# bababyVN/medical-image-segmentation-and-classification

Measured on AMD Instinct MI355X. Metric: images/sec (train step) Attention U-Net 256x256 bs=32/GPU, higher is better.
Workload: dtype bf16; 1 GPU; AttentionUNet 256x256 train step (fwd+BCE+bwd+clip+AdamW), bs=32/GPU, NHWC bf16 activations, fp32 master weights; global_batch=32, parallelism=dp1, hip_graph=False, wgrad_side_stream=True, plan_replay=C (mi355_plan_run)

## Files before the change

### include/mi355conv.h

```cpp
#ifndef MI355CONV_H_
#define MI355CONV_H_

#include <stdint.h>

#ifdef __cplusplus
extern "C" {
#endif

typedef struct ihipStream_t* mi355_stream_t;

enum { MI355_F32 = 0, MI355_BF16 = 1, MI355_F16 = 2 };
enum { MI355_OK = 0, MI355_ERR_ARG = -1, MI355_ERR_UNSUPPORTED = -2, MI355_ERR_RUNTIME = -3 };

int mi355_version(void);
const char* mi355_last_error(void);


int mi355_pack_input_nchw(const float* x, void* y, int N, int C, int H, int W, int Cpad, int dtype,
                          mi355_stream_t s);
int mi355_pack_input_im2col3(const float* x, void* y, int N, int C, int H, int W, int dtype, mi355_stream_t s);
int mi355_unpack_output_nchw(const void* x, float* y, int N, int C, int H, int W, int ld, int dtype,
                             mi355_stream_t s);
int mi355_pack_nchw(const float* x, void* y, int N, int C, int H, int W, int ld, int dtype, mi355_stream_t s);

// ... 6 lines not shown
int mi355_conv2d_igemm(const void* in, const void* wk, const float* bias, void* out,
                       int N, int Hi, int Wi, int Ci, int ldi,
                       int Ho, int Wo, int Co, int ldo,
                       int KH, int KW, int mul, int kmul, int off, int div, int up,
                       int accumulate, float* stats, int dtype, mi355_stream_t s);
int mi355_conv2d_igemm_variant(int Hi, int Wi, int Ci, int Ho, int Wo, int Co, int KH, int KW, int mul, int kmul, int off,
                               int div, int up, int dtype);
int mi355_conv2d_igemm_variant_n(int N, int Hi, int Wi, int Ci, int Ho, int Wo, int Co, int KH, int KW, int mul, int kmul,
                                 int off, int div, int up, int dtype);
int mi355_conv2d_igemm_dma_tile(int N, int Ho, int Wo, int Ci, int Co);
int mi355_conv2d_igemm_generic_tile(int N, int Ho, int Wo, int Co);
int mi355_conv2d_igemm_stat_rows(int N, int Hi, int Wi, int Ci, int Ho, int Wo, int Co, int KH, int KW,
                                 int mul, int kmul, int off, int div, int up, int dtype);
int mi355_conv2d_igemm_pool2_ok(int N, int Hi, int Wi, int Ci, int Ho, int Wo, int Co, int KH, int KW,
                                int mul, int kmul, int off, int div, int up, int dtype);
const char* mi355_conv2d_igemm_kernel_name(int N, int Hi, int Wi, int Ci, int Ho, int Wo, int Co, int KH, int KW,
                                           int mul, int kmul, int off, int div, int up, int dtype);

int mi355_conv2d_wgrad_splits(int N, int Ho, int Wo, int Ci, int Co, int KH, int KW);
int mi355_conv2d_wgrad_variant(int N, int Ho, int Wo, int KH, int KW, int stride, int pad, int dtype);
const char* mi355_conv2d_wgrad_kernel_name(int N, int Ho, int Wo, int Ci, int Co, int KH, int KW, int stride, int pad, int dtype);
int mi355_conv2d_wgrad(const void* x, const void* dy, float* ws, int splits,
                       int N, int Hi, int Wi, int Ci, int ldx,
                       int Ho, int Wo, int Co, int ldy,
                       int KH, int KW, int stride, int pad, int up, int dtype, mi355_stream_t s);
int mi355_conv2d_wgrad_multi_ok(int N, int Ho, int Wo, int dtype);
int mi355_conv2d_wgrad_multi(const void* x0, const void* dy0, const void* x1, const void* dy1, const void* x2, const void* dy2,
                             const void* x3, const void* dy3, const void* x4, const void* dy4, const void* x5, const void* dy5,
                             int napp, float* ws, int splits, int N, int Hi, int Wi, int Ci, int ldx, int Ho, int Wo, int Co,
                             int ldy, int up, int dtype, mi355_stream_t s);
// ... 256 lines not shown
```

### medical-image-segmentation-and-classification_amd/csrc/conv3x3_halo.hpp

```cpp
#pragma once
#include <type_traits>

#include "common.hpp"
#include "conv3x3_tile.hpp"

template <int TH, int TW> struct HaloRwCfg {
  static constexpr int BN = 64;
  static constexpr int NPIX = (TH + 2) * (TW + 2);
  static constexpr int P_INSTR = (NPIX + 15) / 16;
  static constexpr int PATCH_BYTES = P_INSTR * 1024;
  static constexpr int STAGE_BYTES = 3 * BN * 64;
  static constexpr int NS = 3;
  static constexpr int RING = 2 * PATCH_BYTES + NS * STAGE_BYTES;
  static constexpr int C_BYTES = TH * TW * (BN * 2 + 16);
  static constexpr int EPI_BYTES = C_BYTES + 2 * 2 * BN * 4;
  static constexpr int LDS_BYTES = RING > EPI_BYTES ? RING : EPI_BYTES;
};

template <typename T, int TH, int TW>
__global__ __launch_bounds__(256, 2) void conv3x3_halo_rw_kernel(const ConvArgs a) {
  static_assert(sizeof(T) == 2, "bf16 / fp16 only");
  typedef HaloRwCfg<TH, TW> Cfg;
  constexpr int BN = 64, BK = 32, EPC = 8, BM = TH * TW;
  static_assert(BM == 256 && TW % 16 == 0, "tile must hold 256 pixels in rows of 16-pixel blocks");
  constexpr int PH = TH + 2, PW = TW + 2, NPIX = PH * PW;
  constexpr int PIXB = BK * 2;
  constexpr int P_INSTR = Cfg::P_INSTR;
  constexpr int P_IT = (P_INSTR + 3) / 4;
  constexpr int PATCH_BYTES = Cfg::PATCH_BYTES;
  constexpr int SLAB = BN * PIXB, STAGE = Cfg::STAGE_BYTES, NS = Cfg::NS;
  constexpr int B_IT = 3;
  constexpr int WM = 2, WN = 2, WTM = BM / WM, WTN = BN / WN;
  constexpr int RW = WTM / TW, XB = TW / 16;
  constexpr int MB = RW * XB, NB = WTN / 16;
  constexpr int C_PITCH = BN * 2 + 16;
  extern __shared__ __attribute__((aligned(16))) unsigned char lds[];
// ... 159 lines not shown
    }
    if constexpr (STATS) {
#pragma unroll
      for (int nb = 0; nb < NB; ++nb)
#pragma unroll
        for (int r = 0; r < 4; ++r) {
          const float s1 = row16_sum(sm[nb][r >> 1][r & 1]), s2 = row16_sum(sq[nb][r >> 1][r & 1]);
          if (l16 == 0) {
            red[(wm * 2 + 0) * BN + wn * WTN + nb * 16 + 4 * c4 + r] = s1;
            red[(wm * 2 + 1) * BN + wn * WTN + nb * 16 + 4 * c4 + r] = s2;
          }
        }
    }
  };
  using Yes = std::true_type;
  if (a.stats) {
    if (a.relu) finish(Yes{}, Yes{}); else finish(No{}, Yes{});
  } else {
    if (a.relu) finish(Yes{}, No{}); else finish(No{}, No{});
  }
  __syncthreads();
  fold_tile_stats<WM, BN>(a, red, tid, tile);
  constexpr int CPRC = BN / EPC;
  if (a.pool2) {
    const int Ho2 = a.Ho >> 1, Wo2 = a.Wo >> 1;
    for (int id = tid; id < (BM / 4) * CPRC; id += 256) {
      const int g = id / CPRC, c = id - g * CPRC;
      const int gy = g / (TW / 2), gx = g - gy * (TW / 2);
      float sum[EPC];
#pragma unroll
      for (int e = 0; e < EPC; ++e) sum[e] = 0.f;
#pragma unroll
      for (int dy = 0; dy < 2; ++dy)
#pragma unroll
        for (int dx = 0; dx < 2; ++dx) {
          const int row = (2 * gy + dy) * TW + 2 * gx + dx;
          const Vec16<T> v = *reinterpret_cast<const Vec16<T>*>(lds + row * C_PITCH + c * 16);
// ... 4 lines not shown
      Vec16<T> v;
      if (a.accumulate) {
        const Vec16<T> o = ld16<T>(p);
#pragma unroll
        for (int e = 0; e < EPC; ++e) v.v[e] = from_f32<T>(sum[e] + to_f32<T>(o.v[e]));
      } else {
#pragma unroll
        for (int e = 0; e < EPC; ++e) v.v[e] = from_f32<T>(sum[e]);
      }
      st16<T>(p, v);
    }
    return;
  }
  constexpr int NST = BM * CPRC / 256;
  static_assert(NST * 256 == BM * CPRC, "whole store rounds");
  auto addr = [&](int it) __attribute__((always_inline)) {
    const int id = tid + it * 256, row = id / CPRC, c = id - row * CPRC;
    const int py = row / TW, px = row - py * TW;
    return out + ((size_t)(n * a.Ho + y0 + py) * a.Wo + x0 + px) * a.ldo + n0 + c * EPC;
  };
  if (a.accumulate) {
    Vec16<T> old[NST];
#pragma unroll
    for (int it = 0; it < NST; ++it) old[it] = ld16<T>(addr(it));
#pragma unroll
    for (int it = 0; it < NST; ++it) {
      const int id = tid + it * 256, row = id / CPRC, c = id - row * CPRC;
      Vec16<T> v = *reinterpret_cast<const Vec16<T>*>(lds + row * C_PITCH + c * 16);
#pragma unroll
      for (int e = 0; e < EPC; ++e) v.v[e] = from_f32<T>(to_f32<T>(v.v[e]) + to_f32<T>(old[it].v[e]));
      st16<T>(addr(it), v);
    }
  } else {
#pragma unroll
    for (int it = 0; it < NST; ++it) {
      const int id = tid + it * 256, row = id / CPRC, c = id - row * CPRC;
      st16<T>(addr(it), *reinterpret_cast<const Vec16<T>*>(lds + row * C_PITCH + c * 16));
    }
  }
}

template <typename T, int TH, int TW>
static int launch_halo_rw(const ConvArgs& a, hipStream_t s) {
  const int grid = a.N * (a.Ho / TH) * (a.Wo / TW) * (a.Co / 64);
  return launch_with_lds<conv3x3_halo_rw_kernel<T, TH, TW>, HaloRwCfg<TH, TW>::LDS_BYTES>("conv3x3_halo_rw", grid, 256, s, a);
}
```

### medical-image-segmentation-and-classification_amd/csrc/conv3x3_halo_pp128.hpp

```cpp
#pragma once
#include <type_traits>

#include "common.hpp"
#include "conv3x3_tile.hpp"

struct HaloPp128Cfg {
  static constexpr int TH = 16, TW = 32, HTH = 8, BN = 128;
  static constexpr int PWL = 36;
  static constexpr int NPIX = (TH + 2) * PWL;
  static constexpr int P_INSTR = (NPIX + 15) / 16;
  static constexpr int PATCH_BYTES = P_INSTR * 1024;
  static constexpr int STAGE_BYTES = 3 * BN * 64;
  static constexpr int NS = 3;
  static constexpr int NPB = 2;
  static constexpr int RING = NPB * PATCH_BYTES + NS * STAGE_BYTES;
  static constexpr int C_BYTES = HTH * TW * (BN * 2 + 16);
  static constexpr int EPI_BYTES = 2 * C_BYTES + 2 * 2 * 2 * BN * 4;
  static constexpr int LDS_BYTES = RING > EPI_BYTES ? RING : EPI_BYTES;
};

template <typename T>
__global__ __launch_bounds__(512) void conv3x3_halo_pp128_kernel(const ConvArgs a) {
  static_assert(sizeof(T) == 2, "bf16 / fp16 only");
  typedef HaloPp128Cfg Cfg;
  constexpr int TH = Cfg::TH, TW = Cfg::TW, HTH = Cfg::HTH;
  constexpr int BN = Cfg::BN, BK = 32, EPC = 8, HBM = HTH * TW;
  constexpr int PW = TW + 2, PWL = Cfg::PWL, NPIX = Cfg::NPIX;
  constexpr int PIXB = BK * 2;
  constexpr int P_INSTR = Cfg::P_INSTR;
  constexpr int P_IT = P_INSTR / 8;
  static_assert(P_INSTR == 8 * P_IT + 1, "one left-over piece");
  constexpr int PATCH_BYTES = Cfg::PATCH_BYTES;
  constexpr int SLAB = BN * PIXB, STAGE = Cfg::STAGE_BYTES;
  constexpr int WN = 2, WTM = HBM / 2, WTN = BN / WN;
  constexpr int RW = HTH, XB = 1;
  constexpr int MB = RW * XB, NB = WTN / 16;
  constexpr int NPR = RW + 2;
  constexpr int C_PITCH = BN * 2 + 16;
// ... 186 lines not shown
      for (int nb = 0; nb < NB; ++nb) t += acc[mb][nb];
    reinterpret_cast<f32x4*>(a.out)[tid + 512 * blockIdx.x] = t;
    return;
  }
#endif
  T* __restrict__ out = reinterpret_cast<T*>(a.out);
  struct alignas(8) Pack4 { T v[4]; };
  unsigned char* const ctile = lds + half * Cfg::C_BYTES;
  float* const red = reinterpret_cast<float*>(lds + 2 * Cfg::C_BYTES);
  auto finish = [&](auto relu_tag, auto stats_tag) __attribute__((always_inline)) {
    constexpr bool RELU = decltype(relu_tag)::value, STATS = decltype(stats_tag)::value;
    f32x2 sm[NB][2], sq[NB][2];
    f32x4 bias4[NB];
#pragma unroll
    for (int nb = 0; nb < NB; ++nb) {
      bias4[nb] = a.bias ? *reinterpret_cast<const f32x4*>(a.bias + n0 + wn * WTN + nb * 16 + 4 * c4) : f32x4{0.f, 0.f, 0.f, 0.f};
#pragma unroll
      for (int j = 0; j < 2; ++j) { sm[nb][j] = f32x2{0.f, 0.f}; sq[nb][j] = f32x2{0.f, 0.f}; }
    }
#pragma unroll
    for (int mb = 0; mb < MB; ++mb) {
      const int row = mb * TW + wm * 16 + l16;
#pragma unroll
      for (int nb = 0; nb < NB; ++nb) {
        Pack4 pk;
#pragma unroll
        for (int r = 0; r < 4; ++r) {
          const float v = acc[mb][nb][r] + bias4[nb][r];
          pk.v[r] = from_f32<T>(RELU ? __builtin_amdgcn_fmed3f(v, 0.f, INFINITY) : v);
        }
        if constexpr (STATS) {
// ... 9 lines not shown
    }
    if constexpr (STATS) {
#pragma unroll
      for (int nb = 0; nb < NB; ++nb)
#pragma unroll
        for (int r = 0; r < 4; ++r) {
          const float s1 = row16_sum(sm[nb][r >> 1][r & 1]), s2 = row16_sum(sq[nb][r >> 1][r & 1]);
          if (l16 == 0) {
            red[((half * 2 + wm) * 2 + 0) * BN + wn * WTN + nb * 16 + 4 * c4 + r] = s1;
            red[((half * 2 + wm) * 2 + 1) * BN + wn * WTN + nb * 16 + 4 * c4 + r] = s2;
          }
        }
    }
  };
  auto finish_any = [&]() __attribute__((always_inline)) {
    if (a.stats) {
      if (a.relu) finish(Yes{}, Yes{}); else finish(No{}, Yes{});
    } else {
      if (a.relu) finish(Yes{}, No{}); else finish(No{}, No{});
    }
  };
  finish_any();
  __syncthreads();
  fold_tile_stats<4, BN>(a, red, tid, tile);
  constexpr int CPRC = BN / EPC;
  constexpr int BM = TH * TW;
  if (a.pool2) {
    const int Ho2 = a.Ho >> 1, Wo2 = a.Wo >> 1;
    for (int id = tid; id < (BM / 4) * CPRC; id += 512) {
      const int g = id / CPRC, c = id - g * CPRC;
      const int gy = g / (TW / 2), gx = g - gy * (TW / 2);
      float sum[EPC];
#pragma unroll
      for (int e = 0; e < EPC; ++e) sum[e] = 0.f;
#pragma unroll
      for (int dy = 0; dy < 2; ++dy)
#pragma unroll
        for (int dx = 0; dx < 2; ++dx) {
          const int row = (2 * gy + dy) * TW + 2 * gx + dx;
          const Vec16<T> v = *reinterpret_cast<const Vec16<T>*>(lds + (row / HBM) * Cfg::C_BYTES + (row % HBM) * C_PITCH + c * 16);
#pragma unroll
// ... 16 lines not shown
  for (int id = tid; id < BM * CPRC; id += 512) {
    const int row = id / CPRC, c = id - row * CPRC;
    const int py = row / TW, px = row - py * TW;
    T* p = out + ((size_t)(n * a.Ho + y0 + py) * a.Wo + x0 + px) * a.ldo + n0 + c * EPC;
    Vec16<T> v = *reinterpret_cast<const Vec16<T>*>(lds + (row / HBM) * Cfg::C_BYTES + (row % HBM) * C_PITCH + c * 16);
    if (a.accumulate) {
      const Vec16<T> o = ld16<T>(p);
#pragma unroll
      for (int e = 0; e < EPC; ++e) v.v[e] = from_f32<T>(to_f32<T>(v.v[e]) + to_f32<T>(o.v[e]));
    }
    st16<T>(p, v);
  }
}

template <typename T>
static int launch_halo_pp128(const ConvArgs& a, hipStream_t s) {
  const int grid = a.N * (a.Ho / HaloPp128Cfg::TH) * (a.Wo / HaloPp128Cfg::TW) * (a.Co / HaloPp128Cfg::BN);
  return launch_with_lds<conv3x3_halo_pp128_kernel<T>, HaloPp128Cfg::LDS_BYTES>("conv3x3_halo_pp128", grid, 512, s, a);
}
```

### medical-image-segmentation-and-classification_amd/csrc/conv3x3_tile.hpp

```cpp
#pragma once
#include "common.hpp"

struct HaloTile { int sp, n, y0, x0, n0; };
template <int TH, int TW, int BN> __device__ __forceinline__ HaloTile halo_tile(const ConvArgs& a) {
  const int NT = a.Co / BN, TXN = a.Wo / TW, TYN = a.Ho / TH;
  int t = xcd_tile(blockIdx.x, gridDim.x);
  const int nt = t % NT; t /= NT;
  const int sp = t;
  const int tx = t % TXN; t /= TXN;
  const int ty = t % TYN;
  return {sp, t / TYN, ty * TH, tx * TW, nt * BN};
}

template <typename T> __device__ __forceinline__ size_t weight_row_offset(int row, size_t wrow, int slot) {
  return (size_t)row * wrow + (slot ^ (((row >> 2) & 1) << 1)) * (16 / sizeof(T));
}
__device__ __forceinline__ int tap_index(bool flip, int ph, int pw) { return flip ? (2 - ph) * 3 + (2 - pw) : ph * 3 + pw; }

template <int ROWS, int BN> __device__ __forceinline__ void fold_tile_stats(const ConvArgs& a, const float* red, int tid, const HaloTile& t) {
  if (a.stats && tid < 2 * BN) {
    const int q = tid / BN, c = tid - q * BN;
    float v = 0.f;
#pragma unroll
    for (int w = 0; w < ROWS; ++w) v += red[(w * 2 + q) * BN + c];
    a.stats[((size_t)t.sp * 2 + q) * a.Co + t.n0 + c] = v;
  }
}

template <auto KERNEL, int LDS_BYTES, typename... Args>
static int launch_with_lds(const char* name, int grid, int block, hipStream_t s, const Args&... args) {
  static const hipError_t configured = hipFuncSetAttribute((const void*)KERNEL, hipFuncAttributeMaxDynamicSharedMemorySize, LDS_BYTES);
  if (configured != hipSuccess) MI355_FAIL((int)configured, "%s: cannot reserve %d B of LDS: %s", name, LDS_BYTES, hipGetErrorString(configured));
  hipLaunchKernelGGL(KERNEL, dim3(grid), dim3(block), LDS_BYTES, s, args...);
  MI355_LAUNCH_CHECK();
  return MI355_OK;
}
```

### medical-image-segmentation-and-classification_amd/csrc/conv_igemm.hip

```cpp
#include "common.hpp"
#include <stdlib.h>

struct ConvArgs {
  const void* in;
  const void* wk;
  const float* bias;
  void* out;
  int N, Hi, Wi, Ci, ldi;
  int Ho, Wo, Co, ldo;
  int KH, KW;
  int mul, kmul, off, dshift, up;
  int accumulate;
  int relu;
  int pool2;
  float* stats;
  int M;
  int HoWo;
  int Hlog, Wlog;
};

template <typename T> struct Frag;
template <> struct Frag<bf16_t> {
  static __device__ __forceinline__ void mma(const uint4& a, const uint4& b, f32x16& c) {
    c = __builtin_amdgcn_mfma_f32_32x32x16_bf16(__builtin_bit_cast(bf16x8, a), __builtin_bit_cast(bf16x8, b), c, 0,
                                                0, 0);
  }
};
template <> struct Frag<f16_t> {
  static __device__ __forceinline__ void mma(const uint4& a, const uint4& b, f32x16& c) {
    c = mfma_32x32x16<f16_t>(__builtin_bit_cast(bf16x8, a), __builtin_bit_cast(bf16x8, b), c);
  }
};
template <> struct Frag<float> {
// ... 476 lines not shown
    return n;
  }();
  return cus;
}
struct Switches {
  int force_generic = getenv("MI355_IGEMM_VARIANT") ? atoi(getenv("MI355_IGEMM_VARIANT")) == 0 : 0;
  int halo_pp = env_int("MI355_HALO_PP", 0);
  int pp128 = env_int("MI355_HALO_PP128", 1), pp128_min_ci = env_int("MI355_HALO_PP128_MINCI", 256);
  int pp128_fill = env_int("MI355_PP128_FILL", 80);
  int ws64 = env_int("MI355_WS64", 1), ws128 = env_int("MI355_WS128", 1);
  long long ws_min_tiles = getenv("MI355_WS64_MIN_TILES") ? atoll(getenv("MI355_WS64_MIN_TILES")) : 4ll * device_cus();
  int ws128_tile_mult = env_int("MI355_WS128_TILE_MULT", 6);
  int gemm256 = env_int("MI355_GEMM256", 1);
  long long gemm256_min_tiles = getenv("MI355_GEMM256_MIN_TILES") ? atoll(getenv("MI355_GEMM256_MIN_TILES")) : 128;
  int dma_smallgrid = env_int("MI355_DMA_SMALLGRID", 1);
};
static const Switches& switches() { static const Switches sw{}; return sw; }

static bool halo_family(IgemmVariant v) {
  return v == IG_HALO_8x32 || v == IG_HALO_16x16 || v == IG_HALO_PP || v == IG_HALO_PP128 || v == IG_WS64 || v == IG_WS128;
}
static bool image_fits_descriptor(int Hi, int Wi, int ldi, int esz) { return (long long)Hi * Wi * ldi * esz < (1ll << 31); }

static int small_grid_tile_n(long long M, int Co, bool to32) {
  const long long rows = (M + 127) / 128;
  int bn = Co % 128 == 0 ? 128 : (Co % 64 == 0 ? 64 : 32);
  if (switches().dma_smallgrid) {
    const int cus = device_cus();
    if (bn == 128 && rows * (Co / 128) * 2 <= cus) bn = 64;
    if (bn == 64 && to32 && rows * (Co / 64) * 2 <= cus) bn = 32;
// ... 113 lines not shown
#undef IG_KERNEL

#define GEOM_PARAMS int Hi, int Wi, int Ci, int Ho, int Wo, int Co, int KH, int KW, int mul, int kmul, int off, int div, int up, int dtype
#define GEOM_SHAPE(N) ConvShape{N, Hi, Wi, Ci, Ho, Wo, Co, KH, KW, mul, kmul, off, div, up, dtype}
extern "C" int mi355_conv2d_igemm_variant(GEOM_PARAMS) { return (int)choose(GEOM_SHAPE(1)).shape_variant; }
extern "C" int mi355_conv2d_igemm_variant_n(int N, GEOM_PARAMS) { return (int)choose(GEOM_SHAPE(N)).variant; }
extern "C" int mi355_conv2d_igemm_stat_rows(int N, GEOM_PARAMS) { return choose(GEOM_SHAPE(N)).stat_rows; }
extern "C" int mi355_conv2d_igemm_pool2_ok(int N, GEOM_PARAMS) { return choose(GEOM_SHAPE(N)).pool2; }
extern "C" int mi355_conv2d_igemm_dma_tile(int N, int Ho, int Wo, int Ci, int Co) { return small_grid_tile_n((long long)N * Ho * Wo, Co, Ci % 64 == 0); }
extern "C" int mi355_conv2d_igemm_generic_tile(int N, int Ho, int Wo, int Co) { return small_grid_tile_n((long long)N * Ho * Wo, Co, true); }
extern "C" const char* mi355_conv2d_igemm_kernel_name(int N, GEOM_PARAMS) {
  static thread_local char name[IG_NAME_LEN];
  const ConvShape s = GEOM_SHAPE(N); const ConvChoice c = choose(s);
  const int rc = dispatch_dtype(dtype, "conv2d_igemm_kernel_name", [&](auto tag) { return launch_or_name<decltype(tag)>(c, conv_args(s), nullptr, name); });
  return rc == MI355_OK ? name : nullptr;
}

extern "C" int mi355_conv2d_igemm(const void* in, const void* wk, const float* bias, void* out, int N, int Hi, int Wi,
                                  int Ci, int ldi, int Ho, int Wo, int Co, int ldo, int KH, int KW, int mul, int kmul,
                                  int off, int div, int up, int accumulate, float* stats, int dtype, mi355_stream_t s) {
  MI355_CHECK_ARG(in && wk && out, "conv2d_igemm: null pointer");
  MI355_CHECK_ARG(N > 0 && Hi > 0 && Wi > 0 && Ho > 0 && Wo > 0 && KH > 0 && KW > 0, "conv2d_igemm: bad extent");
  MI355_CHECK_ARG(div == 1 || div == 2 || div == 4, "conv2d_igemm: div must be 1, 2 or 4 (got %d)", div);
  MI355_CHECK_ARG(Co % 32 == 0, "conv2d_igemm: Co=%d must be a multiple of 32", Co);
  MI355_CHECK_ARG(ldi >= Ci && ldo >= Co, "conv2d_igemm: channel stride smaller than channel count");
  MI355_CHECK_ARG((long long)N * Ho * Wo < (1ll << 31) && (long long)N * Hi * Wi < (1ll << 31),
                  "conv2d_igemm: pixel count overflows int32");
  MI355_CHECK_ARG(dtype == MI355_BF16 || dtype == MI355_F16 || dtype == MI355_F32, "conv2d_igemm: unknown dtype %d", dtype);
  const int esz = dtype_is_2byte(dtype) ? 2 : 4;
  MI355_CHECK_ARG(((uintptr_t)in % 16) == 0 && ((uintptr_t)wk % 16) == 0 && ((uintptr_t)out % 16) == 0 &&
// ... 22 lines not shown
```

### medical-image-segmentation-and-classification_amd/mi355/graph.py

```python
from __future__ import annotations

import ctypes
import os
import struct
from typing import List, Optional

import torch
import torch.nn as nn

from .lib import lib, DTYPE_CODE

BN_EPS_DEFAULT = 1e-5
CPAD = 32
FUSE_POOL = os.environ.get("MI355_FUSE_POOL", "1") != "0"
FUSE_POOL_BWD = os.environ.get("MI355_FUSE_POOL_BWD", "1") != "0"
FUSE_GATE_BWD = os.environ.get("MI355_FUSE_GATE_BWD", "1") != "0"
FUSE_HEAD = os.environ.get("MI355_FUSE_HEAD", "1") != "0"
STEM_IM2COL = os.environ.get("MI355_STEM_IM2COL", "1") != "0"
SIDE_COLSUM = os.environ.get("MI355_SIDE_COLSUM", "1") != "0"
BN_ACT_WINDOWS = os.environ.get("MI355_BN_ACT_WINDOWS", "1") != "0"
STATIC_PACKS = os.environ.get("MI355_STATIC_PACKS", "1") != "0"
BN_ACT_WINDOWS_RES = os.environ.get("MI355_BN_ACT_WINDOWS_RES", "1") != "0"
FUSE_RESIDUAL = os.environ.get("MI355_FUSE_RESIDUAL", "1") != "0"
DEFER_POST = os.environ.get("MI355_DEFER_POST", "1") != "0"


class T:
    __slots__ = ("buf", "off", "N", "H", "W", "C", "ld", "_ng", "_grad", "parent", "_written", "name", "_bn", "_post_uses", "_post_seen", "_post_pending")

    def __init__(self, buf, off, N, H, W, C, ld, parent=None):
        self.buf, self.off = buf, off
        self.N, self.H, self.W, self.C, self.ld = N, H, W, C, ld
        self._ng = False
        self._grad = None
        self.parent = parent
        self._written = False
        self.name = ""
        self._bn = None
        self._post_uses = 0
        self._post_seen = 0
        self._post_pending = []

    @property
    def needs_grad(self):
        return self._ng

    @needs_grad.setter
    def needs_grad(self, v):
        self._ng = bool(v)
        if v and self.parent is not None:
            self.parent._ng = True

    @property
    def M(self):
        return self.N * self.H * self.W

# ... 295 lines not shown
        self.device = torch.device(device)
        self.dtype = dtype
        self.code = DTYPE_CODE[dtype]
        self.esz = 4 if dtype == torch.float32 else 2
        self.epc = 16 // self.esz
        self.training = training
        self.want_grad = want_grad and training
        self.explain = bool(explain) and not training
        self.cam = None
        self.pre: List[Launch] = []
        self.fwd: List[Launch] = []
        self.bwd: List[Launch] = []
        self._rules = []
        self._conv_uses = {}
        self._pending_wgrad = {}
        self._post_operands = []
        self.multi_wgrad = os.environ.get("MI355_WGRAD_MULTI", "1") != "0"
        self.keep = []
        self.ws_need = {"bytes": 0, "f32": 0}
        self._packs = {}
        self._pack_table = []
        self._grad_first = {}
        self.params_seen = []
        self.grad_params = []
        self.zero_grad_params = []
        self.input = None
        self.output = None
        self.dout = None
        self.bn_momentum = 0.1
        self.acts = []
# ... 32 lines not shown
    def grad_of(self, t):
        if t._grad is None:
            if isinstance(t, V):
                t._grad = V(self.f32(t.B * t.F), t.B, t.F)
            elif t.parent is not None:
                pg = self.grad_of(t.parent)
                t._grad = T(pg.buf, t.off, t.N, t.H, t.W, t.C, pg.ld, parent=pg)
            else:
                t._grad = T(self._alloc(t.M * t.ld), 0, t.N, t.H, t.W, t.C, t.ld)
        return t._grad

    def acc_flag(self, t):
        g = self.grad_of(t)
        root = g.parent if (not isinstance(g, V) and g.parent is not None) else g
        was = g._written or root._written
        g._written = True
        if root is not g and g.C == root.C:
            root._written = True
        return 1 if was else 0

    def grad_written(self, t):
        g = t._grad
        if g is None:
            parent = None if isinstance(t, V) else t.parent
            return bool(parent is not None and parent._grad is not None and parent._grad._written)
        root = g.parent if (not isinstance(g, V) and g.parent is not None) else g
        return bool(g._written or root._written)

    def mark_full_written(self, t):
        g = self.grad_of(t)
# ... 152 lines not shown
            elif self.param_grad(conv.weight):
                splits = lib.mi355_conv2d_wgrad_splits(x.N, Ho, Wo, x.C, Co, k, k)
                ws = self.ws_bytes(splits * Co * k * k * x.C * 4)
                self.bwd.append(Launch("mi355_conv2d_wgrad", x, dy, ws, splits, x.N, x.H, x.W, x.C, x.ld, Ho, Wo, Co, dy.ld,
                                       k, k, s, p, 1 if up else 0, self.code, flops=flops, nbytes=nbytes, side=True,
                                       tag=self.wgrad_tag(Co, x.C, k, s, Ho, Wo, x.N, p), cus=self.wgrad_cus(x.N, Ho, Wo, x.C, Co, k, s, p, splits)))
                ref, beta = self.pgrad(conv.weight)
                self.bwd.append(Launch("mi355_conv2d_wgrad_reduce", ws, splits, ref, Co, x.C, conv.in_channels, k, k, 0, beta, side=True))
            if conv.bias is not None and self.param_grad(conv.bias) and not bias_done:
                self.bias_grad_from(dy, conv.bias)
            if x.needs_grad:
                acc = self.acc_flag(x)
                xg = self.grad_of(x)
                hg, wg = (2 * x.H, 2 * x.W) if up else (x.H, x.W)
                dgeom = (x.N, Ho, Wo, Co, hg, wg, x.C, k, k, 1, -1, p, s, 0)
                if not up:
                    self.bwd.append(self.igemm(dy, wb, None, xg, dgeom, acc, flops=flops, nbytes=nbytes))
                elif lib.mi355_conv2d_igemm_pool2_ok(*dgeom, self.code):
                    self.bwd.append(self.igemm(dy, wb, None, xg, dgeom, 4 | (1 if acc else 0), flops=flops, nbytes=nbytes))
                else:
                    tmp = self.new_tensor(x.N, hg, wg, x.C)
                    self.bwd.append(self.igemm(dy, wb, None, tmp, dgeom, 0, flops=flops, nbytes=nbytes))
                    self.bwd.append(Launch("mi355_upsample2_bwd", tmp, tmp.ld, xg, xg.ld, x.N, x.H, x.W, x.C, acc, self.code))
        return y, bwd, stat_rows

    def _emit_multi_wgrad(self, conv, pend, Ho, Wo, Co, k, up, flops, nbytes):
        x0 = pend[0][0]
        n = len(pend)
        splits = lib.mi355_conv2d_wgrad_splits(x0.N * n, Ho, Wo, x0.C, Co, k, k)
        ws = self.ws_bytes(splits * Co * k * k * x0.C * 4)
        ops = []
        for i in range(6):
            ops += list(pend[i]) if i < n else [None, None]
        self.bwd.append(Launch("mi355_conv2d_wgrad_multi", *ops, n, ws, splits, x0.N, x0.H, x0.W, x0.C, x0.ld, Ho, Wo, Co,
                               pend[0][1].ld, 1 if up else 0, self.code, flops=flops * n, nbytes=nbytes * n, side=True,
                               tag=self.wgrad_tag(Co, x0.C, k, 1, Ho, Wo, x0.N, 1), cus=self.wgrad_cus(x0.N, Ho, Wo, x0.C, Co, k, 1, 1, splits)))
        ref, beta = self.pgrad(conv.weight)
        self.bwd.append(Launch("mi355_conv2d_wgrad_reduce", ws, splits, ref, Co, x0.C, conv.in_channels, k, k, 0, beta, side=True))

# ... 92 lines not shown
        ops = (da, da.ld if da is not None else 0, dp, dp.ld, y, y.ld)
        co, dims = (st["mean"], st["invstd"], st["scale"], st["shift"]), (y.N, y.H, y.W, C, self.code)
        self.bwd.append(Launch("mi355_bn_bwd_reduce_pool2", *ops, *co, part, *dims, nbytes=int((1.25 + (da is not None)) * y.M * C * self.esz)))
        sums = self._bn_param_grads(bn, part, min(nb, lib.mi355_bn_bwd_reduce_pool2_rows(y.M)))
        dy = self.grad_of(y)
        self._zero_bias_grad(rec.bias)
        self.bwd.append(Launch("mi355_bn_bwd_apply_pool2", *ops, bn.weight, *co, sums, dy, dy.ld, *dims,
                               nbytes=int((2.25 + (da is not None)) * y.M * C * self.esz)))
        return dy

    def _bn_bwd_plain(self, rec, da):
        y, bn, st, act = rec.y, rec.bn, rec.st, rec.act
        dres_to, post_to = (None, rec.res) if rec.post else (rec.res, None)
        C = bn.num_features
        nb = lib.mi355_rowreduce_blocks(y.M)
        part = self.ws_f32(nb * 2 * C)
        am = rec.a if (act and dres_to is not None) else None
        ops = (da, da.ld, am, am.ld if am is not None else 0, y, y.ld)
        co, dims = (st["mean"], st["invstd"], st["scale"], st["shift"]), (y.M, C, 1 if act else 0, self.code)
        self.bwd.append(Launch("mi355_bn_bwd_reduce", *ops, *co, part, *dims, nbytes=(2 + (am is not None)) * y.M * C * self.esz))
        sums = self._bn_param_grads(bn, part, min(nb, lib.mi355_bn_bwd_reduce_rows(y.M)))
        dy = self.grad_of(y)
        ops += (bn.weight, *co, sums, dy, dy.ld)
        dres = None
        if dres_to is not None and dres_to.needs_grad:
            dres = self.new_tensor(y.N, y.H, y.W, C) if self.acc_flag(dres_to) else self.grad_of(dres_to)
        self._zero_bias_grad(rec.bias)
        pg, pacc = None, 0
        if post_to is not None and post_to.needs_grad:
            post_to._post_seen += 1
            pend = post_to._post_pending
            last_one = post_to._post_seen >= post_to._post_uses
            if DEFER_POST and dres is None and not last_one and len(pend) < 4 and all(t.ld == da.ld for t in pend):
                pend.append(da)
            else:
                pacc = self.acc_flag(post_to)
# ... 519 lines not shown
                self.pre.append(pack_launch(live))
        if self.cam is not None:
            kind, y, _ = self.output
            assert kind == "v" and self.dout is not None, "the CAM tap must feed the classifier head"
            self.cam_target = self._alloc(y.B, torch.int32)
            self.bwd.append(Launch("mi355_cam_seed", y, None, y.B, y.F, self.dout, self.cam_target))
        for r in reversed(self._rules):
            r()
        if self.cam is not None:
            t = self.cam
            g = self.grad_of(t)
            assert g._written, "the head's backward did not reach the CAM tap"
            self.cam_lowres = self.f32(t.N * t.H * t.W)
            self.bwd.append(Launch("mi355_gradcam", t, t.ld, g, g.ld, t.N, t.H * t.W, t.C, self.code, self.cam_lowres))
        assert not self._pending_wgrad, "a shared convolution's weight gradient is still waiting for an application's backward"
        assert not self.want_grad or all(not t._post_pending and t._post_seen == (t._post_uses if t.needs_grad else 0)
                                         for t in self._post_operands), "a post_add operand's gradient lacks an application's incoming gradient"
        if os.environ.get("MI355_TAIL_ON_MAIN", "1") != "0":
            tail = []
            for l in reversed(self.bwd):
                if not l.side:
                    break
                tail.append(l)
            need = 0
            for l in tail:
                if l.name == "mi355_conv2d_wgrad_reduce":
                    need = max(need, int(l.arg("splits")) * int(l.arg("Co")) * int(l.arg("Ci")) * int(l.arg("KH")) * int(l.arg("KW")) * 4)
            own = self._alloc(need, torch.uint8) if need else None
            if all(not isinstance(a, Ws) or (a.kind == "bytes" and own is not None) for l in tail for a in l.args):
                for l in tail:
# ... 9 lines not shown
```

Before: 2185 images/s.

## Fuse BatchNorm backward reductions into data-gradient conv epilogue

Adds bsum variants of the halo conv kernels that, while storing the data gradient, also read the BN input activation and accumulate the per-channel sum of gradient and gradient times normalized input (with ReLU masking) into per-tile partials. The graph builder routes eligible conv dgrad launches to these kernels and skips the separate bn_bwd_reduce launch. This removes a full re-read of the gradient and activation tensors and one launch per eligible BN layer. In exchange the conv epilogue gains an extra activation load and an extra reduction with a barrier, which may add register pressure, and fusion is limited to non-accumulating, non-residual cases.

```diff
diff --git a/include/mi355conv.h b/include/mi355conv.h
--- a/include/mi355conv.h
+++ b/include/mi355conv.h
@@ -44,6 +44,16 @@
                                  int mul, int kmul, int off, int div, int up, int dtype);
 int mi355_conv2d_igemm_pool2_ok(int N, int Hi, int Wi, int Ci, int Ho, int Wo, int Co, int KH, int KW,
                                 int mul, int kmul, int off, int div, int up, int dtype);
+int mi355_conv2d_igemm_bsum_rows(int N, int Hi, int Wi, int Ci, int Ho, int Wo, int Co, int KH, int KW,
+                                 int mul, int kmul, int off, int div, int up, int dtype, int accumulate);
+int mi355_conv2d_igemm_bsum(const void* in, const void* wk, void* out,
+                            int N, int Hi, int Wi, int Ci, int ldi,
+                            int Ho, int Wo, int Co, int ldo,
+                            int KH, int KW, int mul, int kmul, int off, int div, int up,
+                            int accumulate,
+                            const void* bn_y, int bn_ldy, const float* mean, const float* invstd,
+                            const float* mscale, const float* mshift, int act, float* partial,
+                            int dtype, mi355_stream_t s);
 const char* mi355_conv2d_igemm_kernel_name(int N, int Hi, int Wi, int Ci, int Ho, int Wo, int Co, int KH, int KW,
                                            int mul, int kmul, int off, int div, int up, int dtype);
 
diff --git a/medical-image-segmentation-and-classification_amd/csrc/conv3x3_halo.hpp b/medical-image-segmentation-and-classification_amd/csrc/conv3x3_halo.hpp
--- a/medical-image-segmentation-and-classification_amd/csrc/conv3x3_halo.hpp
+++ b/medical-image-segmentation-and-classification_amd/csrc/conv3x3_halo.hpp
@@ -17,9 +17,10 @@
   static constexpr int LDS_BYTES = RING > EPI_BYTES ? RING : EPI_BYTES;
 };
 
-template <typename T, int TH, int TW>
-__global__ __launch_bounds__(256, 2) void conv3x3_halo_rw_kernel(const ConvArgs a) {
+template <typename T, int TH, int TW, typename Args>
+__device__ __forceinline__ void conv3x3_halo_rw_body(const Args& a) {
   static_assert(sizeof(T) == 2, "bf16 / fp16 only");
+  constexpr bool BWD_SUMS = std::is_same<Args, ConvSumArgs>::value;
   typedef HaloRwCfg<TH, TW> Cfg;
   constexpr int BN = 64, BK = 32, EPC = 8, BM = TH * TW;
   static_assert(BM == 256 && TW % 16 == 0, "tile must hold 256 pixels in rows of 16-pixel blocks");
@@ -209,13 +210,15 @@
     }
   };
   using Yes = std::true_type;
-  if (a.stats) {
+  if constexpr (BWD_SUMS) {
+    finish(No{}, No{});
+  } else if (a.stats) {
     if (a.relu) finish(Yes{}, Yes{}); else finish(No{}, Yes{});
   } else {
     if (a.relu) finish(Yes{}, No{}); else finish(No{}, No{});
   }
   __syncthreads();
-  fold_tile_stats<WM, BN>(a, red, tid, tile);
+  if constexpr (!BWD_SUMS) fold_tile_stats<WM, BN>(a, red, tid, tile);
   constexpr int CPRC = BN / EPC;
   if (a.pool2) {
     const int Ho2 = a.Ho >> 1, Wo2 = a.Wo >> 1;
@@ -250,6 +253,31 @@
   }
   constexpr int NST = BM * CPRC / 256;
   static_assert(NST * 256 == BM * CPRC, "whole store rounds");
+  if constexpr (BWD_SUMS) {
+    static_assert(Cfg::C_BYTES + 4 * 2 * BN * 4 <= Cfg::LDS_BYTES, "red[4 waves][2][BN] behind the C tile");
+    const T* __restrict__ yb = reinterpret_cast<const T*>(a.bsum_y);
+    const int c = tid % CPRC;
+    auto pixel = [&](int it) __attribute__((always_inline)) {
+      const int row = (tid + it * 256) / CPRC;
+      const int py = row / TW, px = row - py * TW;
+      return (size_t)(n * a.Ho + y0 + py) * a.Wo + x0 + px;
+    };
+    Vec16<T> yv[NST];
+#pragma unroll
+    for (int it = 0; it < NST; ++it) yv[it] = ld16<T>(yb + pixel(it) * a.bsum_ldy + n0 + c * EPC);
+    BwdSums<T> bs;
+    bs.init(a, n0 + c * EPC);
+#pragma unroll
+    for (int it = 0; it < NST; ++it) {
+      const int row = (tid + it * 256) / CPRC;
+      const Vec16<T> v = *reinterpret_cast<const Vec16<T>*>(lds + row * C_PITCH + c * 16);
+      st16<T>(out + pixel(it) * a.ldo + n0 + c * EPC, v);
+      bsum_pin(yv[it]);
+      bs.add(v, yv[it]);
+    }
+    bs.template fold_store<CPRC, 4, BN>(a, red, tid, tile.sp, n0);
+    return;
+  }
   auto addr = [&](int it) __attribute__((always_inline)) {
     const int id = tid + it * 256, row = id / CPRC, c = id - row * CPRC;
     const int py = row / TW, px = row - py * TW;
@@ -277,7 +305,15 @@
 }
 
 template <typename T, int TH, int TW>
-static int launch_halo_rw(const ConvArgs& a, hipStream_t s) {
+__global__ __launch_bounds__(256, 2) void conv3x3_halo_rw_kernel(const ConvArgs a) { conv3x3_halo_rw_body<T, TH, TW, ConvArgs>(a); }
+template <typename T, int TH, int TW>
+__global__ __launch_bounds__(256, 2) void conv3x3_halo_rw_bsum_kernel(const ConvSumArgs a) { conv3x3_halo_rw_body<T, TH, TW, ConvSumArgs>(a); }
+
+template <typename T, int TH, int TW, typename Args>
+static int launch_halo_rw(const Args& a, hipStream_t s) {
   const int grid = a.N * (a.Ho / TH) * (a.Wo / TW) * (a.Co / 64);
-  return launch_with_lds<conv3x3_halo_rw_kernel<T, TH, TW>, HaloRwCfg<TH, TW>::LDS_BYTES>("conv3x3_halo_rw", grid, 256, s, a);
+  if constexpr (std::is_same<Args, ConvSumArgs>::value)
+    return launch_with_lds<conv3x3_halo_rw_bsum_kernel<T, TH, TW>, HaloRwCfg<TH, TW>::LDS_BYTES>("conv3x3_halo_rw_bsum", grid, 256, s, a);
+  else
+    return launch_with_lds<conv3x3_halo_rw_kernel<T, TH, TW>, HaloRwCfg<TH, TW>::LDS_BYTES>("conv3x3_halo_rw", grid, 256, s, a);
 }
diff --git a/medical-image-segmentation-and-classification_amd/csrc/conv3x3_halo_pp128.hpp b/medical-image-segmentation-and-classification_amd/csrc/conv3x3_halo_pp128.hpp
--- a/medical-image-segmentation-and-classification_amd/csrc/conv3x3_halo_pp128.hpp
+++ b/medical-image-segmentation-and-classification_amd/csrc/conv3x3_halo_pp128.hpp
@@ -19,9 +19,10 @@
   static constexpr int LDS_BYTES = RING > EPI_BYTES ? RING : EPI_BYTES;
 };
 
-template <typename T>
-__global__ __launch_bounds__(512) void conv3x3_halo_pp128_kernel(const ConvArgs a) {
+template <typename T, typename Args>
+__device__ __forceinline__ void conv3x3_halo_pp128_body(const Args& a) {
   static_assert(sizeof(T) == 2, "bf16 / fp16 only");
+  constexpr bool BWD_SUMS = std::is_same<Args, ConvSumArgs>::value;
   typedef HaloPp128Cfg Cfg;
   constexpr int TH = Cfg::TH, TW = Cfg::TW, HTH = Cfg::HTH;
   constexpr int BN = Cfg::BN, BK = 32, EPC = 8, HBM = HTH * TW;
@@ -238,7 +239,8 @@
     f32x4 bias4[NB];
 #pragma unroll
     for (int nb = 0; nb < NB; ++nb) {
-      bias4[nb] = a.bias ? *reinterpret_cast<const f32x4*>(a.bias + n0 + wn * WTN + nb * 16 + 4 * c4) : f32x4{0.f, 0.f, 0.f, 0.f};
+      if constexpr (BWD_SUMS) bias4[nb] = f32x4{0.f, 0.f, 0.f, 0.f};
+      else bias4[nb] = a.bias ? *reinterpret_cast<const f32x4*>(a.bias + n0 + wn * WTN + nb * 16 + 4 * c4) : f32x4{0.f, 0.f, 0.f, 0.f};
 #pragma unroll
       for (int j = 0; j < 2; ++j) { sm[nb][j] = f32x2{0.f, 0.f}; sq[nb][j] = f32x2{0.f, 0.f}; }
     }
@@ -278,7 +280,9 @@
     }
   };
   auto finish_any = [&]() __attribute__((always_inline)) {
-    if (a.stats) {
+    if constexpr (BWD_SUMS) {
+      finish(No{}, No{});
+    } else if (a.stats) {
       if (a.relu) finish(Yes{}, Yes{}); else finish(No{}, Yes{});
     } else {
       if (a.relu) finish(Yes{}, No{}); else finish(No{}, No{});
@@ -286,9 +290,78 @@
   };
   finish_any();
   __syncthreads();
-  fold_tile_stats<4, BN>(a, red, tid, tile);
+  if constexpr (!BWD_SUMS) fold_tile_stats<4, BN>(a, red, tid, tile);
   constexpr int CPRC = BN / EPC;
   constexpr int BM = TH * TW;
+  if constexpr (BWD_SUMS) {
+    static_assert(2 * Cfg::C_BYTES + 8 * 2 * BN * 4 <= Cfg::LDS_BYTES, "red[8 waves][2][BN] behind the C tiles");
+    const T* __restrict__ yb = reinterpret_cast<const T*>(a.bsum_y);
+    const int c = tid % CPRC;
+    BwdSums<T> bs;
+    if (a.pool2) {
+      const int Wo2 = a.Wo >> 1;
+      constexpr int NST = (BM / 4) * CPRC / 512;
+      const size_t org = (size_t)(n * (a.Ho >> 1) + (y0 >> 1)) * Wo2 + (x0 >> 1);
+      const T* const yt = yb + org * a.bsum_ldy + n0;
+      T* const ot = out + org * a.ldo + n0;
+      auto pixel = [&](int it) __attribute__((always_inline)) {
+        const int g = (tid + it * 512) / CPRC;
+        const int gy = g / (TW / 2), gx = g - gy * (TW / 2);
+        return (unsigned)(gy * Wo2 + gx);
+      };
+      Vec16<T> yv[NST];
+#pragma unroll
+      for (int it = 0; it < NST; ++it) yv[it] = ld16<T>(yt + (pixel(it) * (unsigned)a.bsum_ldy + (unsigned)(c * EPC)));
+      bs.init(a, n0 + c * EPC);
+#pragma unroll
+      for (int it = 0; it < NST; ++it) {
+        const int g = (tid + it * 512) / CPRC;
+        const int gy = g / (TW / 2), gx = g - gy * (TW / 2);
+        float sum[EPC];
+#pragma unroll
+        for (int e = 0; e < EPC; ++e) sum[e] = 0.f;
+#pragma unroll
+        for (int dy = 0; dy < 2; ++dy)
+#pragma unroll
+          for (int dx = 0; dx < 2; ++dx) {
+            const int row = (2 * gy + dy) * TW + 2 * gx + dx;
+            const Vec16<T> v = *reinterpret_cast<const Vec16<T>*>(lds + (row / HBM) * Cfg::C_BYTES + (row % HBM) * C_PITCH + c * 16);
+#pragma unroll
+            for (int e = 0; e < EPC; ++e) sum[e] += to_f32<T>(v.v[e]);
+          }
+        Vec16<T> v;
+#pragma unroll
+        for (int e = 0; e < EPC; ++e) v.v[e] = from_f32<T>(sum[e]);
+        st16<T>(ot + (pixel(it) * (unsigned)a.ldo + (unsigned)(c * EPC)), v);
+        bsum_pin(yv[it]);
+        bs.add(v, yv[it]);
+      }
+    } else {
+      constexpr int NST = BM * CPRC / 512;
+      const size_t org = (size_t)(n * a.Ho + y0) * a.Wo + x0;
+      const T* const yt = yb + org * a.bsum_ldy + n0;
+      T* const ot = out + org * a.ldo + n0;
+      auto pixel = [&](int it) __attribute__((always_inline)) {
+        const int row = (tid + it * 512) / CPRC;
+        const int py = row / TW, px = row - py * TW;
+        return (unsigned)(py * a.Wo + px);
+      };
+      Vec16<T> yv[NST];
+#pragma unroll
+      for (int it = 0; it < NST; ++it) yv[it] = ld16<T>(yt + (pixel(it) * (unsigned)a.bsum_ldy + (unsigned)(c * EPC)));
+      bs.init(a, n0 + c * EPC);
+#pragma unroll
+      for (int it = 0; it < NST; ++it) {
+        const int row = (tid + it * 512) / CPRC;
+        const Vec16<T> v = *reinterpret_cast<const Vec16<T>*>(lds + (row / HBM) * Cfg::C_BYTES + (row % HBM) * C_PITCH + c * 16);
+        st16<T>(ot + (pixel(it) * (unsigned)a.ldo + (unsigned)(c * EPC)), v);
+        bsum_pin(yv[it]);
+        bs.add(v, yv[it]);
+      }
+    }
+    bs.template fold_store<CPRC, 8, BN>(a, red, tid, tile.sp, n0);
+    return;
+  }
   if (a.pool2) {
     const int Ho2 = a.Ho >> 1, Wo2 = a.Wo >> 1;
     for (int id = tid; id < (BM / 4) * CPRC; id += 512) {
@@ -335,7 +408,15 @@
 }
 
 template <typename T>
-static int launch_halo_pp128(const ConvArgs& a, hipStream_t s) {
+__global__ __launch_bounds__(512) void conv3x3_halo_pp128_kernel(const ConvArgs a) { conv3x3_halo_pp128_body<T, ConvArgs>(a); }
+template <typename T>
+__global__ __launch_bounds__(512) void conv3x3_halo_pp128_bsum_kernel(const ConvSumArgs a) { conv3x3_halo_pp128_body<T, ConvSumArgs>(a); }
+
+template <typename T, typename Args>
+static int launch_halo_pp128(const Args& a, hipStream_t s) {
   const int grid = a.N * (a.Ho / HaloPp128Cfg::TH) * (a.Wo / HaloPp128Cfg::TW) * (a.Co / HaloPp128Cfg::BN);
-  return launch_with_lds<conv3x3_halo_pp128_kernel<T>, HaloPp128Cfg::LDS_BYTES>("conv3x3_halo_pp128", grid, 512, s, a);
+  if constexpr (std::is_same<Args, ConvSumArgs>::value)
+    return launch_with_lds<conv3x3_halo_pp128_bsum_kernel<T>, HaloPp128Cfg::LDS_BYTES>("conv3x3_halo_pp128_bsum", grid, 512, s, a);
+  else
+    return launch_with_lds<conv3x3_halo_pp128_kernel<T>, HaloPp128Cfg::LDS_BYTES>("conv3x3_halo_pp128", grid, 512, s, a);
 }
diff --git a/medical-image-segmentation-and-classification_amd/csrc/conv3x3_tile.hpp b/medical-image-segmentation-and-classification_amd/csrc/conv3x3_tile.hpp
--- a/medical-image-segmentation-and-classification_amd/csrc/conv3x3_tile.hpp
+++ b/medical-image-segmentation-and-classification_amd/csrc/conv3x3_tile.hpp
@@ -27,6 +27,69 @@
   }
 }
 
+template <typename V> __device__ __forceinline__ void bsum_pin(V& v) {
+  static_assert(sizeof(V) == 16, "a 16-byte load result");
+  typedef unsigned u32x4_t __attribute__((ext_vector_type(4)));
+  u32x4_t w = __builtin_bit_cast(u32x4_t, v);
+  asm volatile("" : "+v"(w) : : "memory");
+  v = __builtin_bit_cast(V, w);
+}
+template <typename T> struct BwdSums {
+  static constexpr int EPC = 8;
+  float q0[EPC], q1[EPC], mu[EPC], is[EPC], ms[EPC], mt[EPC];
+  bool act;
+  __device__ __forceinline__ void init(const ConvSumArgs& a, int c0) {
+    act = a.bsum_act != 0;
+#pragma unroll
+    for (int e = 0; e < EPC; ++e) {
+      q0[e] = q1[e] = 0.f;
+      mu[e] = a.bsum_mean[c0 + e];
+      is[e] = a.bsum_invstd[c0 + e];
+      ms[e] = a.bsum_mscale[c0 + e];
+      mt[e] = a.bsum_mshift[c0 + e];
+    }
+  }
+  __device__ __forceinline__ void add(const Vec16<T>& g, const Vec16<T>& y) {
+#pragma unroll
+    for (int e = 0; e < EPC; ++e) {
+      float gg = to_f32<T>(g.v[e]);
+      const float xf = to_f32<T>(y.v[e]);
+      if (act) {
+        const bool on = __builtin_fmaf(xf, ms[e], mt[e]) > 0.f;
+        if (!on) gg = 0.f;
+      }
+      q0[e] += gg;
+      q1[e] += gg * (xf - mu[e]) * is[e];
+    }
+  }
+  template <int CPRC, int NW, int BN> __device__ __forceinline__ void fold_store(const ConvSumArgs& a, float* red, int tid, int row, int n0) {
+    static_assert(CPRC * EPC == BN && 64 % CPRC == 0 && 2 * BN <= NW * 64, "a chunk per lane % CPRC, a thread per (q, channel)");
+    const int lane = tid & 63, wave = tid >> 6;
+#pragma unroll
+    for (int e = 0; e < EPC; ++e)
+#pragma unroll
+      for (int m = CPRC; m < 64; m <<= 1) {
+        q0[e] += __shfl_xor(q0[e], m);
+        q1[e] += __shfl_xor(q1[e], m);
+      }
+    if (lane < CPRC) {
+#pragma unroll
+      for (int e = 0; e < EPC; ++e) {
+        red[(wave * 2 + 0) * BN + lane * EPC + e] = q0[e];
+        red[(wave * 2 + 1) * BN + lane * EPC + e] = q1[e];
+      }
+    }
+    __syncthreads();
+    if (tid < 2 * BN) {
+      const int q = tid / BN, c = tid - q * BN;
+      float v = 0.f;
+#pragma unroll
+      for (int w = 0; w < NW; ++w) v += red[(w * 2 + q) * BN + c];
+      a.bsum_part[((size_t)row * 2 + q) * a.Co + n0 + c] = v;
+    }
+  }
+};
+
 template <auto KERNEL, int LDS_BYTES, typename... Args>
 static int launch_with_lds(const char* name, int grid, int block, hipStream_t s, const Args&... args) {
   static const hipError_t configured = hipFuncSetAttribute((const void*)KERNEL, hipFuncAttributeMaxDynamicSharedMemorySize, LDS_BYTES);
diff --git a/medical-image-segmentation-and-classification_amd/csrc/conv_igemm.hip b/medical-image-segmentation-and-classification_amd/csrc/conv_igemm.hip
--- a/medical-image-segmentation-and-classification_amd/csrc/conv_igemm.hip
+++ b/medical-image-segmentation-and-classification_amd/csrc/conv_igemm.hip
@@ -17,6 +17,17 @@
   int M;
   int HoWo;
   int Hlog, Wlog;
+};
+
+struct ConvSumArgs : ConvArgs {
+  const void* bsum_y;
+  int bsum_ldy;
+  const float* bsum_mean;
+  const float* bsum_invstd;
+  const float* bsum_mscale;
+  const float* bsum_mshift;
+  int bsum_act;
+  float* bsum_part;
 };
 
 template <typename T> struct Frag;
@@ -523,6 +534,7 @@
   int gemm256 = env_int("MI355_GEMM256", 1);
   long long gemm256_min_tiles = getenv("MI355_GEMM256_MIN_TILES") ? atoll(getenv("MI355_GEMM256_MIN_TILES")) : 128;
   int dma_smallgrid = env_int("MI355_DMA_SMALLGRID", 1);
+  int bsum_pp128 = env_int("MI355_BSUM_PP128", 1), bsum_rw = env_int("MI355_BSUM_RW", 1);
 };
 static const Switches& switches() { static const Switches sw{}; return sw; }
 
@@ -666,6 +678,63 @@
   const ConvShape s = GEOM_SHAPE(N); const ConvChoice c = choose(s);
   const int rc = dispatch_dtype(dtype, "conv2d_igemm_kernel_name", [&](auto tag) { return launch_or_name<decltype(tag)>(c, conv_args(s), nullptr, name); });
   return rc == MI355_OK ? name : nullptr;
+}
+
+static int bsum_rows(const ConvShape& s, const ConvChoice& c, int flags) {
+  if (!dtype_is_2byte(s.dtype) || (flags & 3)) return 0;
+  const bool pool2 = (flags >> 2) & 1;
+  switch (c.variant) {
+    case IG_HALO_PP128: return switches().bsum_pp128 ? s.N * (s.Ho / 16) * (s.Wo / 32) : 0;
+    case IG_HALO_8x32: return switches().bsum_rw && !pool2 ? s.N * (s.Ho / 8) * (s.Wo / 32) : 0;
+    case IG_HALO_16x16: return switches().bsum_rw && !pool2 ? s.N * (s.Ho / 16) * (s.Wo / 16) : 0;
+    default: return 0;
+  }
+}
+extern "C" int mi355_conv2d_igemm_bsum_rows(int N, GEOM_PARAMS, int accumulate) {
+  const ConvShape s = GEOM_SHAPE(N);
+  return bsum_rows(s, choose(s), accumulate);
+}
+
+extern "C" int mi355_conv2d_igemm_bsum(const void* in, const void* wk, void* out, int N, int Hi, int Wi, int Ci, int ldi, int Ho, int Wo,
+                                       int Co, int ldo, int KH, int KW, int mul, int kmul, int off, int div, int up, int accumulate,
+                                       const void* bn_y, int bn_ldy, const float* mean, const float* invstd, const float* mscale,
+                                       const float* mshift, int act, float* partial, int dtype, mi355_stream_t s) {
+  MI355_CHECK_ARG(in && wk && out && bn_y && mean && invstd && mscale && mshift && partial, "conv2d_igemm_bsum: null pointer");
+  MI355_CHECK_ARG(N > 0 && Hi > 0 && Wi > 0 && Ho > 0 && Wo > 0, "conv2d_igemm_bsum: bad extent");
+  MI355_CHECK_ARG(div == 1 || div == 2 || div == 4, "conv2d_igemm_bsum: div must be 1, 2 or 4 (got %d)", div);
+  MI355_CHECK_ARG(ldi >= Ci && ldo >= Co && bn_ldy >= Co, "conv2d_igemm_bsum: channel stride smaller than channel count");
+  MI355_CHECK_ARG((long long)N * Ho * Wo < (1ll << 31) && (long long)N * Hi * Wi < (1ll << 31), "conv2d_igemm_bsum: pixel count overflows int32");
+  MI355_CHECK_ARG(((uintptr_t)in % 16) == 0 && ((uintptr_t)wk % 16) == 0 && ((uintptr_t)out % 16) == 0 && ((uintptr_t)bn_y % 16) == 0 &&
+                      (ldi * 2) % 16 == 0 && (ldo * 2) % 16 == 0 && (bn_ldy * 2) % 16 == 0,
+                  "conv2d_igemm_bsum: pointers / channel strides must be 16-byte aligned");
+  const ConvShape shape = GEOM_SHAPE(N);
+  const ConvChoice c = choose(shape);
+  MI355_CHECK_ARG(bsum_rows(shape, c, accumulate) > 0,
+                  "conv2d_igemm_bsum: no kernel forms the BatchNorm backward sums for this shape / dtype / epilogue (mi355_conv2d_igemm_bsum_rows == 0)");
+  MI355_CHECK_ARG(16ll * Wo * (ldo > bn_ldy ? ldo : bn_ldy) < (1ll << 31), "conv2d_igemm_bsum: 16 rows of %d pixels at a channel stride of %d overflow a 32-bit offset",
+                  Wo, ldo > bn_ldy ? ldo : bn_ldy);
+  MI355_CHECK_ARG(image_fits_descriptor(Hi, Wi, ldi, 2), "conv2d_igemm_bsum: an image of %d x %d pixels at a channel stride of %d is 2 GiB or more", Hi, Wi, ldi);
+  ConvSumArgs a = {};
+  static_cast<ConvArgs&>(a) = conv_args(shape);
+  a.in = in; a.wk = wk; a.bias = nullptr; a.out = out;
+  a.ldi = ldi; a.ldo = ldo;
+  a.pool2 = (accumulate >> 2) & 1;
+  a.bsum_y = bn_y; a.bsum_ldy = bn_ldy;
+  a.bsum_mean = mean; a.bsum_invstd = invstd; a.bsum_mscale = mscale; a.bsum_mshift = mshift;
+  a.bsum_act = act ? 1 : 0;
+  a.bsum_part = partial;
+  return dispatch_dtype(dtype, "conv2d_igemm_bsum", [&](auto tag) {
+    using T = decltype(tag);
+    if constexpr (sizeof(T) == 2) {
+      switch (c.variant) {
+        case IG_HALO_PP128: return launch_halo_pp128<T>(a, (hipStream_t)s);
+        case IG_HALO_8x32: return launch_halo_rw<T, 8, 32>(a, (hipStream_t)s);
+        case IG_HALO_16x16: return launch_halo_rw<T, 16, 16>(a, (hipStream_t)s);
+        default: break;
+      }
+    }
+    return (int)MI355_ERR_ARG;
+  });
 }
 
 extern "C" int mi355_conv2d_igemm(const void* in, const void* wk, const float* bias, void* out, int N, int Hi, int Wi,
diff --git a/medical-image-segmentation-and-classification_amd/mi355/graph.py b/medical-image-segmentation-and-classification_amd/mi355/graph.py
--- a/medical-image-segmentation-and-classification_amd/mi355/graph.py
+++ b/medical-image-segmentation-and-classification_amd/mi355/graph.py
@@ -22,11 +22,12 @@
 STATIC_PACKS = os.environ.get("MI355_STATIC_PACKS", "1") != "0"
 BN_ACT_WINDOWS_RES = os.environ.get("MI355_BN_ACT_WINDOWS_RES", "1") != "0"
 FUSE_RESIDUAL = os.environ.get("MI355_FUSE_RESIDUAL", "1") != "0"
+FUSE_BN_BWD_SUMS = os.environ.get("MI355_FUSE_BN_BWD_SUMS", "1") != "0"
 DEFER_POST = os.environ.get("MI355_DEFER_POST", "1") != "0"
 
 
 class T:
-    __slots__ = ("buf", "off", "N", "H", "W", "C", "ld", "_ng", "_grad", "parent", "_written", "name", "_bn", "_post_uses", "_post_seen", "_post_pending")
+    __slots__ = ("buf", "off", "N", "H", "W", "C", "ld", "_ng", "_grad", "parent", "_written", "name", "_bn", "_post_uses", "_post_seen", "_post_pending", "_bsum")
 
     def __init__(self, buf, off, N, H, W, C, ld, parent=None):
         self.buf, self.off = buf, off
@@ -40,6 +41,7 @@
         self._post_uses = 0
         self._post_seen = 0
         self._post_pending = []
+        self._bsum = None
 
     @property
     def needs_grad(self):
@@ -365,6 +367,7 @@
         self._rules = []
         self._conv_uses = {}
         self._pending_wgrad = {}
+        self._bsum_open = []
         self._post_operands = []
         self.multi_wgrad = os.environ.get("MI355_WGRAD_MULTI", "1") != "0"
         self.keep = []
@@ -427,6 +430,7 @@
         g = self.grad_of(t)
         root = g.parent if (not isinstance(g, V) and g.parent is not None) else g
         was = g._written or root._written
+        assert not was or getattr(t, "_bsum", None) is None, "a second gradient contribution to an activation whose BatchNorm sums the first one's launch formed"
         g._written = True
         if root is not g and g.C == root.C:
             root._written = True
@@ -609,7 +613,18 @@
                 xg = self.grad_of(x)
                 hg, wg = (2 * x.H, 2 * x.W) if up else (x.H, x.W)
                 dgeom = (x.N, Ho, Wo, Co, hg, wg, x.C, k, k, 1, -1, p, s, 0)
-                if not up:
+                dflags = None if up and not lib.mi355_conv2d_igemm_pool2_ok(*dgeom, self.code) else (4 if up else 0) | (1 if acc else 0)
+                rows = self._bsum_rows(x, dgeom, dflags) if dflags is not None else 0
+                if rows:
+                    rec = x._bn
+                    part = self.f32(rows * 2 * x.C)
+                    self.bwd.append(Launch("mi355_conv2d_igemm_bsum", dy, wb, xg, *dgeom[:4], dy.ld, *dgeom[4:7], xg.ld, *dgeom[7:], dflags,
+                                           rec.y, rec.y.ld, rec.st["mean"], rec.st["invstd"], rec.st["scale"], rec.st["shift"], 1 if rec.act else 0,
+                                           part, self.code, tag=self.igemm_tag(dgeom).replace("_kernel", "_bsum_kernel"), flops=flops,
+                                           nbytes=nbytes + x.M * x.C * self.esz))
+                    x._bsum = (part, rows)
+                    self._bsum_open.append(x)
+                elif not up:
                     self.bwd.append(self.igemm(dy, wb, None, xg, dgeom, acc, flops=flops, nbytes=nbytes))
                 elif lib.mi355_conv2d_igemm_pool2_ok(*dgeom, self.code):
                     self.bwd.append(self.igemm(dy, wb, None, xg, dgeom, 4 | (1 if acc else 0), flops=flops, nbytes=nbytes))
@@ -618,6 +633,18 @@
                     self.bwd.append(self.igemm(dy, wb, None, tmp, dgeom, 0, flops=flops, nbytes=nbytes))
                     self.bwd.append(Launch("mi355_upsample2_bwd", tmp, tmp.ld, xg, xg.ld, x.N, x.H, x.W, x.C, acc, self.code))
         return y, bwd, stat_rows
+
+    def _bsum_rows(self, x, dgeom, flags):
+        rec = x._bn
+        if not FUSE_BN_BWD_SUMS or self.esz != 2 or (flags & 1) or rec is None or rec.a is not x or x.parent is not None:
+            return 0
+        if (rec.res is not None or rec.post or rec.pool_out is not None or rec.head is not None or rec.pool_dp is not None
+                or rec.head_dz is not None or not self.training):
+            return 0
+        touching = sum(1 for l in self.fwd if isinstance(l, Launch) and any(isinstance(v, T) and v.buf is x.buf for v in l.args))
+        if touching != 2 or any(not isinstance(l, Launch) for l in self.fwd):
+            return 0
+        return max(0, lib.mi355_conv2d_igemm_bsum_rows(*dgeom, self.code, flags))
 
     def _emit_multi_wgrad(self, conv, pend, Ho, Wo, Co, k, up, flops, nbytes):
         x0 = pend[0][0]
@@ -740,12 +767,19 @@
         dres_to, post_to = (None, rec.res) if rec.post else (rec.res, None)
         C = bn.num_features
         nb = lib.mi355_rowreduce_blocks(y.M)
-        part = self.ws_f32(nb * 2 * C)
         am = rec.a if (act and dres_to is not None) else None
         ops = (da, da.ld, am, am.ld if am is not None else 0, y, y.ld)
         co, dims = (st["mean"], st["invstd"], st["scale"], st["shift"]), (y.M, C, 1 if act else 0, self.code)
-        self.bwd.append(Launch("mi355_bn_bwd_reduce", *ops, *co, part, *dims, nbytes=(2 + (am is not None)) * y.M * C * self.esz))
-        sums = self._bn_param_grads(bn, part, min(nb, lib.mi355_bn_bwd_reduce_rows(y.M)))
+        fused = rec.a._bsum if rec.a is not None else None
+        if fused is not None:
+            assert am is None and da is rec.a._grad
+            rec.a._bsum = None
+            self._bsum_open.remove(rec.a)
+            sums = self._bn_param_grads(bn, *fused)
+        else:
+            part = self.ws_f32(nb * 2 * C)
+            self.bwd.append(Launch("mi355_bn_bwd_reduce", *ops, *co, part, *dims, nbytes=(2 + (am is not None)) * y.M * C * self.esz))
+            sums = self._bn_param_grads(bn, part, min(nb, lib.mi355_bn_bwd_reduce_rows(y.M)))
         dy = self.grad_of(y)
         ops += (bn.weight, *co, sums, dy, dy.ld)
         dres = None
@@ -1295,6 +1329,7 @@
             self.cam_lowres = self.f32(t.N * t.H * t.W)
             self.bwd.append(Launch("mi355_gradcam", t, t.ld, g, g.ld, t.N, t.H * t.W, t.C, self.code, self.cam_lowres))
         assert not self._pending_wgrad, "a shared convolution's weight gradient is still waiting for an application's backward"
+        assert not self._bsum_open, "a data gradient left BatchNorm backward sums that no layer's backward took"
         assert not self.want_grad or all(not t._post_pending and t._post_seen == (t._post_uses if t.needs_grad else 0)
                                          for t in self._post_operands), "a post_add operand's gradient lacks an application's incoming gradient"
         if os.environ.get("MI355_TAIL_ON_MAIN", "1") != "0":
```

Result: no change. 2198 images/s, median of 6 (+0.6%).
